# Mictronics/multi-sdr-gps-sim

Measured on AMD Instinct MI355X. Metric: IQ Msamples/s @16ch int8, higher is better.
Workload: dtype u64

## Files before the change

### multi-sdr-gps-sim_amd/csrc/gpsiq_chain_kernels.hip

```cpp
#include <hip/hip_runtime.h>

#include "gpsiq_internal.h"
#include "gpsiq_lane.h"

namespace gpsiq {

using lane::Prep;
using lane::Rec;
using lane::Stretch;
using lane::Walker;
using lane::u128;

constexpr int kPrepThreads = 1024;
constexpr int kLaneThreads = 256;
constexpr int kTabMinSeg = 16;

struct ScanR { u128 v; int flag; };
struct ScanD { double v; int flag; };
__device__ inline ScanR scan_join(const ScanR &p, ScanR a) { if (!a.flag) { a.v = p.v + a.v; a.flag = p.flag; } return a; }
__device__ inline ScanD scan_join(const ScanD &p, ScanD a) { if (!a.flag) { a.v = p.v + a.v; a.flag = p.flag; } return a; }
__device__ inline ScanR scan_up(const ScanR &x, int off)
{
    ScanR o;
    const uint64_t hi = __shfl_up((uint64_t) (x.v >> 64), off, 64), lo = __shfl_up((uint64_t) x.v, off, 64);
    o.v = ((u128) hi << 64) | lo; o.flag = __shfl_up(x.flag, off, 64);
    return o;
}
__device__ inline ScanD scan_up(const ScanD &x, int off) { ScanD o; o.v = __shfl_up(x.v, off, 64); o.flag = __shfl_up(x.flag, off, 64); return o; }
template <class S>
__device__ inline void block_scan(S mine, S *s_wave, S *before, S *total)
{
    const int lane = threadIdx.x & 63, wave = threadIdx.x >> 6, nwaves = (int) (blockDim.x >> 6);
    S inc = mine;
    for (int off = 1; off < 64; off <<= 1) {
        const S o = scan_up(inc, off);
        if (lane >= off) inc = scan_join(o, inc);
    }
    S exc = scan_up(inc, 1);
    if (lane == 0) { exc.v = 0; exc.flag = 0; }
    if (lane == 63) s_wave[wave] = inc;
    __syncthreads();
    S acc; acc.v = 0; acc.flag = 0;
    S mine_before = acc;
    for (int w = 0; w < nwaves; ++w) {
        if (w == wave) mine_before = acc;
        acc = scan_join(acc, s_wave[w]);
    }
    *before = scan_join(mine_before, exc);
    *total = acc;
    __syncthreads();
}

__global__ __launch_bounds__(kPrepThreads) void chain_prepare(const char *__restrict__ in_rows, int stride, int nblocks, int nchan, double delt, int nsamp,
                                                              const gpsiq_chain_est_t *__restrict__ start, Prep *__restrict__ prep,
                                                              double *__restrict__ c_before, gpsiq_chain_est_t *__restrict__ end)
{
    auto in_at = [&](size_t k) -> gpsiq_chain_in_t { return *reinterpret_cast<const gpsiq_chain_in_t *>(in_rows + k * (size_t) stride); };
    __shared__ ScanR s_wr[kPrepThreads / 64];
    __shared__ ScanD s_wd[kPrepThreads / 64];
    __shared__ int s_any_seed;
    const int i = blockIdx.x, tid = threadIdx.x;
    u128 Rc = 0;
    double Dc = 0.0, carr0 = 0.0, f_prev0 = 0.0;
    int prn0 = 0;
    bool exact0 = false;
    if (start) {
        const gpsiq_chain_est_t e = start[i];
        Rc = ((u128) e.r_hi << 64) | e.r_lo; Dc = e.drift; carr0 = e.carr; f_prev0 = e.f_carr; prn0 = e.prn; exact0 = (e.flags & GPSIQ_CHAIN_EXACT) != 0;
    }
    if (tid == 0) { c_before[i] = prn0 > 0 ? f_prev0 * delt : 0.0; s_any_seed = 0; }
    int last_prn = prn0;
    double last_f = f_prev0;
    __syncthreads();
    for (int base = 0; base < nblocks; base += kPrepThreads) {
        const int b = base + tid;
        const bool live = b < nblocks;
        gpsiq_chain_in_t d = {0.0, 0.0, 0, 0};
        int prev_prn = 0;
        if (live) {
            d = in_at((size_t) b * nchan + i);
            prev_prn = b > 0 ? in_at((size_t) (b - 1) * nchan + i).prn : prn0;
            if (prev_prn < 0) prev_prn = 0;
        }
        const bool active = live && d.prn > 0;
        const bool cont = active && b == 0 && exact0 && prev_prn == d.prn;
        const bool seed = active && (prev_prn != d.prn || cont);
        const double c = active ? d.f_carr * delt : 0.0;
        const double x_seed = cont ? carr0 : d.carr_phase;
        const u128 adv = active ? lane::advance_units(c, nsamp) : (u128) 0;
        ScanR mine;
        mine.flag = seed ? 1 : 0;
        mine.v = seed ? lane::phase_units(x_seed) + adv : adv;
        ScanR pr, er;
        block_scan(mine, s_wr, &pr, &er);
        const u128 R0 = seed ? lane::phase_units(x_seed) : pr.flag ? pr.v : Rc + pr.v;
        const double r0 = lane::units_to_double(R0);
        double core = 0.0;
        if (active && __builtin_fabs(c) < 0.5) core = lane::drift_core(c, seed ? (x_seed < 1.0 ? x_seed : 0.0) : r0, nsamp);
        ScanD md;
        md.flag = seed ? 1 : 0;
        md.v = core;
        ScanD pd, ed;
        block_scan(md, s_wd, &pd, &ed);
        const double D0 = seed ? 0.0 : pd.flag ? pd.v : Dc + pd.v;
        if (live) {
            Prep p = {0.0, 0.0, 0.0, lane::kSkip, 0};
            if (active) {
                p.c = c;
                p.est = seed ? x_seed : lane::wrap01(r0 + D0);
                p.core = core;
                p.flags = seed ? lane::kSeed : 0;
            }
            prep[(size_t) b * nchan + i] = p;
        }
        if (seed) atomicOr(&s_any_seed, 1);
        const int n_here = nblocks - base < kPrepThreads ? nblocks - base : kPrepThreads;
        __syncthreads();
        Rc = er.flag ? er.v : Rc + er.v;
        Dc = ed.flag ? ed.v : Dc + ed.v;
        {
            const gpsiq_chain_in_t l = in_at((size_t) (base + n_here - 1) * nchan + i);
            last_prn = l.prn > 0 ? l.prn : 0;
            last_f = l.f_carr;
        }
        __syncthreads();
    }
    if (end && tid == 0) {
        gpsiq_chain_est_t e;
        e.r_hi = (uint64_t) (Rc >> 64); e.r_lo = (uint64_t) Rc; e.drift = Dc; e.carr = 0.0; e.f_carr = last_f; e.prn = last_prn;
        e.flags = s_any_seed ? GPSIQ_CHAIN_RESEEDED : 0; e.first_prn = 0; e.reserved = 0;
        end[i] = e;
    }
}

template <int kSeg>
__global__ __launch_bounds__(kLaneThreads) void chain_lanes(const Prep *__restrict__ prep, const double *__restrict__ c_before,
                                                            int nblocks, int nchan, int nsamp, int max_seg, Rec *__restrict__ rec)
{
    constexpr int kBlocks = kLaneThreads / kSeg;
    __shared__ __attribute__((aligned(16))) unsigned char walker_raw[sizeof(Walker) * (kBlocks + 1)];
    Walker *walker = reinterpret_cast<Walker *>(walker_raw);
    constexpr int kEnt = kSeg >= kTabMinSeg ? lane::kEntriesHost : 0;
    __shared__ lane::Cycle cycles[kEnt ? kBlocks * kEnt : 1];
    __shared__ int usable[kBlocks + 1];
    const int groups = (nblocks + kBlocks - 1) / kBlocks;
    const int i = blockIdx.x / groups, b0 = (blockIdx.x % groups) * kBlocks;
    const int tid = threadIdx.x;
    if (tid <= kBlocks) {
        const int b = b0 - 1 + tid;
        double c = 0.0;
        if (b < 0) c = c_before[i];
        else if (b < nblocks) { const Prep p = prep[(size_t) b * nchan + i]; c = (p.flags & lane::kSkip) ? 0.0 : p.c; }
        const bool ok = c != 0.0 && __builtin_fabs(c) < 0.5;
        walker[tid].setup_head(ok ? c : 0.25);
        usable[tid] = ok && !walker[tid].general;
    }
    __syncthreads();
    for (int q = tid; q < (kBlocks + 1) * lane::kTab; q += kLaneThreads) {
        const int w = q / lane::kTab, s = q % lane::kTab;
        if (usable[w] && s > Walker::kLow && s <= (int) (1022 - walker[w].ec)) walker[w].setup_piece(s);
    }
    __syncthreads();
    const int blk = tid / kSeg, t = tid % kSeg, b = b0 + blk;
    const bool live = b < nblocks && usable[blk + 1];
    Prep p = {0.0, 0.0, 0.0, lane::kSkip, 0};
    if (live) p = prep[(size_t) b * nchan + i];
    const bool use_tab = live && kEnt > 0 && __builtin_fabs(p.c) * (double) nsamp > 2.0 * kEnt;
    if (use_tab) {
        for (int k = t; k < kEnt; k += kSeg) {
            lane::Cycle e;
            lane::build_cycle(walker[blk + 1], k, kEnt, &e);
            cycles[kEnt ? blk * kEnt + k : 0] = e;
        }
    }
    __syncthreads();
    int nseg = 0;
    Stretch st;
    st.r_in = 0.0; st.x_out = 0.0; st.x_end = 0.0; st.lo = 0; st.hi = 0; st.n_in = -1; st.n_out = -1; st.ok = 0; st.why = lane::kWhyAddend; st.sigma = 0; st.pad = 0;
    if (live) {
        nseg = lane::stretches(p.c, nsamp, max_seg < kSeg ? max_seg : kSeg);
        if (t < nseg) {
            const Walker *prev = (!(p.flags & lane::kSeed) && usable[blk]) ? &walker[blk] : nullptr;
            lane::walk_stretch(walker[blk + 1], prev, p, nsamp, t, nseg, use_tab ? &cycles[kEnt ? blk * kEnt : 0] : nullptr, kEnt, &st);
        }
    }
    const bool mine = live && t < nseg;
    const bool neg = walker[blk + 1].neg;
    const int64_t grid = neg ? 1 : 2;
    lane::JoinLane jl;
    jl.el = lane::join_identity(); jl.D = 0; jl.fail = 0; jl.pad = 0;
    Stretch before = st;
    before.x_out = __shfl_up(st.x_out, 1, kSeg); before.n_out = __shfl_up(st.n_out, 1, kSeg);
    if (mine) jl = lane::join_lane(before, st, t, grid);
    lane::JoinMap inc = jl.el;
    for (int off = 1; off < kSeg; off <<= 1) {
        lane::JoinMap o;
        o.t0 = __shfl_up(inc.t0, off, kSeg); o.t1 = __shfl_up(inc.t1, off, kSeg);
        if (t >= off) inc = lane::join_compose(o, inc);
    }
// ... 53 lines not shown
```

### multi-sdr-gps-sim_amd/csrc/gpsiq_eval.h

```cpp
#ifndef GPSIQ_EVAL_H
#define GPSIQ_EVAL_H

#include "../../include/gpsiq.h"
#include "gpsiq_lane.h"

namespace gpsiq {
namespace ev {

typedef unsigned __int128 u128;
typedef __int128 i128;

struct DChan {
    double   f_carr;
    double   carr_phase;
    int32_t  prn;
    uint32_t pos;
    double   f_code;
    double   code_phase;
    double   gain;
    uint64_t nav;
    double   start;
};
static_assert(sizeof(DChan) == 64, "DChan is one cache line");
constexpr uint32_t kBadPos = UINT32_C(1) << 31;
// ... 240 lines not shown
        if (c0 != c1) return false;
        if (c0 > (i128) INT64_MAX / 2 || c0 < -((i128) INT64_MAX / 2)) return false;
        *cell = (int64_t) c0;
        return true;
    }
};

enum { kEvalOk = 0, kEvalHost = 1 };
constexpr int kCandCap = 256;

GPSIQ_HD inline int eval_quantize(const DChan &d, double phase, double delt, int nsamp, gpsiq_qchan_t *q)
{
    if (d.prn > 0 && !(phase >= 0.0 && phase <= 1.0)) { gpsiq_qchan_t z; z.carr_phase = 0; z.carr_step = 0; z.code_frac = 0; z.code_step = 0; z.gain = 0.0; z.nav_bits = 0; z.chip0 = 0; z.icode = 0; z.prn = 0; *q = z; return kQStart; }
    const uint64_t seeded = phase_to_fixed(phase == 1.0 ? 0.0 : phase);
    return quantize_dchan(d, delt, nsamp, &seeded, q);
}

template <class Chips, class Emit>
GPSIQ_HD inline int eval_candidates(const DChan &d, const gpsiq_qchan_t &qq, double start, double delt, int nsamp, const Chips &chips, Emit &emit)
{
    const long ns = nsamp;
    if (ns <= 0 || d.prn <= 0) return kEvalOk;
    if (!(start >= 0.0 && start <= 1.0)) return -kQStart;
    const double carr_inc = d.f_carr * delt, code_inc = d.f_code * delt;
    uint64_t seed_off = (phase_to_fixed(start == 1.0 ? 0.0 : start) - qq.carr_phase) & kEvCarrMask;
    if (seed_off > (UINT64_C(1) << (GPSIQ_CARR_FRAC_BITS - 1))) seed_off = (UINT64_C(1) << GPSIQ_CARR_FRAC_BITS) - seed_off;
    const uint64_t w_carr = ((uint64_t) ns << (GPSIQ_CARR_FRAC_BITS - 54)) + (uint64_t) ns / 2 + 4 + seed_off;
    const uint64_t w_code = ((uint64_t) ns << (GPSIQ_CODE_FRAC_BITS - 44)) + (uint64_t) ns / 2 + 4;
    const bool want_c = carr_inc != 0.0 || seed_off != 0;
    if ((want_c && 2 * w_carr + 1 >= (UINT64_C(1) << (GPSIQ_CARR_FRAC_BITS - 9))) || 2 * w_code + 1 >= (UINT64_C(1) << GPSIQ_CODE_FRAC_BITS)) return kEvalHost;
    uint64_t nc = want_c ? next_candidate(qq.carr_phase, (uint64_t) qq.carr_step, GPSIQ_CARR_FRAC_BITS - 9, w_carr, ns, 0) : kNoHit;
    uint64_t nk = next_candidate(qq.code_frac, qq.code_step, GPSIQ_CODE_FRAC_BITS, w_code, ns, 0);
    if (nc == kNoHit && nk == kNoHit) return kEvalOk;
    DriftLite dc, dk;
    bool have_c = false, have_k = false;
    int count_c = 0, count_k = 0;
    const int icode = dchan_icode(d);
    while (nc != kNoHit || nk != kNoHit) {
        const uint64_t n = nc < nk ? nc : nk;
        const bool in_c = nc == n, in_k = nk == n;
        const uint64_t P = (qq.carr_phase + (uint64_t) qq.carr_step * n) & kEvCarrMask;
        const unsigned idx_f = (unsigned) (P >> (GPSIQ_CARR_FRAC_BITS - 9));
        const u128 T = (u128) qq.code_frac + (u128) qq.code_step * n;
        const uint64_t A = (uint64_t) qq.chip0 + (uint64_t) (T >> GPSIQ_CODE_FRAC_BITS);
        const unsigned chip_f = (unsigned) (A % GPSIQ_CA_SEQ_LEN);
        const long per_f = (long) (A / GPSIQ_CA_SEQ_LEN);
        const unsigned neg_f = chips(d.prn, chip_f) ^ dchan_nav_bit(d, ((long) icode + per_f) / 20);
        unsigned idx = idx_f, neg_d = neg_f;
        int64_t cell;
        if (in_c) {
            if (++count_c > kCandCap) return kEvalHost;
            if (!have_c) { dc.setup(carr_inc, 1, start); have_c = true; }
            if (!dc.cell_at((long) n, &cell)) return kEvalHost;
            idx = (unsigned) (cell & 511);
            nc = next_candidate(qq.carr_phase, (uint64_t) qq.carr_step, GPSIQ_CARR_FRAC_BITS - 9, w_carr, ns, (long) n + 1);
        }
        if (in_k) {
            if (++count_k > kCandCap) return kEvalHost;
            if (!have_k) { dk.setup(code_inc, 0, d.code_phase); have_k = true; }
            if (!dk.cell_at((long) n, &cell) || cell < 0) return kEvalHost;
            const unsigned chip_d = (unsigned) (cell % GPSIQ_CA_SEQ_LEN);
            const long per_d = (long) (cell / GPSIQ_CA_SEQ_LEN);
            neg_d = chips(d.prn, chip_d) ^ dchan_nav_bit(d, ((long) icode + per_d) / 20);
            nk = next_candidate(qq.code_frac, qq.code_step, GPSIQ_CODE_FRAC_BITS, w_code, ns, (long) n + 1);
        }
        if (idx != idx_f || neg_d != neg_f) emit((uint32_t) n, (uint16_t) idx, (uint8_t) neg_d);
    }
    return kEvalOk;
}

template <class Chips, class Emit>
GPSIQ_HD inline int eval_chan(const DChan &d, double start, double est, double delt, int nsamp, const Chips &chips, Emit &emit, gpsiq_qchan_t *q)
{
    const int qs = eval_quantize(d, est, delt, nsamp, q);
    if (qs != kQOk) return -qs;
    return eval_candidates(d, *q, start, delt, nsamp, chips, emit);
}

struct Link {
    int64_t t[4];
    int32_t abs;
    int32_t pad;
};
GPSIQ_HD inline Link link_identity() { Link l; l.t[0] = l.t[1] = l.t[2] = l.t[3] = 0; l.abs = 0; l.pad = 0; return l; }
GPSIQ_HD inline Link link_compose(const Link &a, const Link &b)
{
    if (b.abs) return b;
    Link o;
    o.abs = a.abs; o.pad = 0;
    for (int r = 0; r < 4; ++r) {
        const int64_t v = a.t[r];
        const int64_t at = a.abs ? v : (int64_t) r + v;
        o.t[r] = v + b.t[at & 3];
    }
    return o;
}
GPSIQ_HD inline int64_t link_apply(const Link &a, int64_t d) { return a.abs ? a.t[0] : d + a.t[d & 3]; }

GPSIQ_HD inline Link link_element(bool seed_or_unused, int64_t d0, const lane::Rec &prev, double xs, bool *ok)
{
    Link l = link_identity();
    *ok = true;
    if (seed_or_unused) { l.abs = 1; l.t[0] = l.t[1] = l.t[2] = l.t[3] = d0; return l; }
    int64_t J;
    const int64_t grid = prev.info & 0xff;
    if (!prev.ok || grid < 1 || grid > 2 || !lane::exact_units(prev.e, xs, &J)) { *ok = false; l.abs = 1; return l; }
    for (int r = 0; r < 4; ++r) l.t[r] = prev.cum[(r >> (grid - 1)) & 1] + J;
    return l;
}
GPSIQ_HD inline bool link_check(const lane::Rec &r, int64_t d, double *next)
{
    if (!r.ok) return false;
    const int64_t grid = r.info & 0xff;
    if (d < r.lo || d > r.hi || grid < 1 || grid > 2 || (d & (grid - 1))) return false;
    const int p = (int) ((d >> (grid - 1)) & 1);
    if (!(r.ok & (1 << p))) return false;
    double y;
    if (!lane::exact_shift(r.e, d + r.cum[p], &y) || !(y >= 0.0 && y < 1.0)) return false;
    *next = y;
    return true;
}

}
}
#endif
```

### multi-sdr-gps-sim_amd/csrc/gpsiq_eval_kernels.hip

```cpp
#include <hip/hip_runtime.h>

#include <cstdio>
#include <cstdlib>

#include "gpsiq_internal.h"
#include "gpsiq_eval.h"
#include "gpsiq_evalctl.h"

namespace gpsiq {

using ev::DChan;
using ev::Link;
using lane::Rec;

constexpr int kPackThreads = 128;
constexpr int kLinkThreads = 256;
constexpr int kEvalThreads = 128;

__device__ inline long long sum16(long long v)
{
    for (int off = 8; off >= 1; off >>= 1) v += __shfl_xor(v, off, 16);
    return v;
}
__device__ inline unsigned long long wave_max_u64(unsigned long long v)
{
    for (int off = 32; off >= 1; off >>= 1) { const unsigned long long o = __shfl_xor(v, off, 64); v = o > v ? o : v; }
    return v;
}
__device__ inline long long wave_max_i64(long long v)
{
    for (int off = 32; off >= 1; off >>= 1) { const long long o = __shfl_xor(v, off, 64); v = o > v ? o : v; }
    return v;
}

__device__ inline void reduce_params(bool counts, unsigned long long code_step, long long amp, EvalCtrl *ctrl)
{
    const long long blk_amp = sum16(counts ? amp : 0);
    const long long blk_active = sum16(counts ? 1 : 0);
    const unsigned long long ms = wave_max_u64(counts ? code_step : 0);
    const long long ma = wave_max_i64(blk_amp), mc = wave_max_i64(blk_active);
    if ((threadIdx.x & 63) == 0) {
        if (ms > __hip_atomic_load(&ctrl->max_code_step, __ATOMIC_RELAXED, __HIP_MEMORY_SCOPE_AGENT)) atomicMax(&ctrl->max_code_step, ms);
        if (ma > __hip_atomic_load(&ctrl->max_amp, __ATOMIC_RELAXED, __HIP_MEMORY_SCOPE_AGENT)) atomicMax(&ctrl->max_amp, ma);
        if ((int) mc > __hip_atomic_load(&ctrl->max_active, __ATOMIC_RELAXED, __HIP_MEMORY_SCOPE_AGENT)) atomicMax(&ctrl->max_active, (int) mc);
    }
}

constexpr int kPackRows = kPackThreads;
constexpr int kRowWords = (int) (sizeof(gpsiq_chan_t) / 8);
static_assert(sizeof(gpsiq_chan_t) % 8 == 0, "rows are streamed as 8-byte words");
__global__ __launch_bounds__(kPackThreads) void pack_raw(const gpsiq_chan_t *__restrict__ ch, int nblocks, int nchan, double delt,
                                                         DChan *__restrict__ out, EvalCtrl *__restrict__ ctrl)
{
    __shared__ __attribute__((aligned(16))) uint64_t rows[kPackRows * kRowWords];
    constexpr int kBlocksPerWg = kPackThreads / 16;
    const int blk0 = (int) blockIdx.x * kBlocksPerWg;
    const int nblk = nblocks - blk0 < kBlocksPerWg ? nblocks - blk0 : kBlocksPerWg;
    const size_t first = (size_t) blk0 * nchan;
    const int words = nblk > 0 ? nblk * nchan * kRowWords : 0;
    const uint64_t *src = reinterpret_cast<const uint64_t *>(ch + first);
    constexpr int kInFlight = 16;
    for (int w0 = threadIdx.x; w0 < words; w0 += kPackThreads * kInFlight) {
        uint64_t t[kInFlight];
#pragma unroll
        for (int j = 0; j < kInFlight; ++j) { const int w = w0 + j * kPackThreads; t[j] = w < words ? src[w] : 0; }
#pragma unroll
        for (int j = 0; j < kInFlight; ++j) { const int w = w0 + j * kPackThreads; if (w < words) rows[w] = t[j]; }
    }
    __syncthreads();
    const int lb = (int) (threadIdx.x >> 4), i = (int) (threadIdx.x & 15);
    const int b = blk0 + lb;
    const bool live = lb < nblk && i < nchan;
    DChan d;
    d.f_carr = 0.0; d.carr_phase = 0.0; d.prn = 0; d.pos = 0; d.f_code = 0.0; d.code_phase = 0.0; d.gain = 0.0; d.nav = 0; d.start = 0.0;
    if (live) {
        ev::pack_chan(*reinterpret_cast<const gpsiq_chan_t *>(&rows[(size_t) (lb * nchan + i) * kRowWords]), &d);
        out[(size_t) b * nchan + i] = d;
    }
    const double code_inc = d.f_code * delt;
    const bool counts = live && d.prn > 0 && d.prn <= 32 && code_inc > 0.0 && code_inc < 2.0 && d.gain > -ev::kEvMaxGain && d.gain < ev::kEvMaxGain;
    reduce_params(counts, counts ? (unsigned long long) (long long) __builtin_rint(code_inc * 0x1p56) : 0ull,
                  counts ? (long long) (250.0 * __builtin_fabs(d.gain)) : 0ll, ctrl);
}

__global__ __launch_bounds__(kLinkThreads) void chain_link_scan(DChan *__restrict__ chan, const Rec *__restrict__ rec, int b0, int nb, int nchan,
                                                                double delt, LinkCarry *__restrict__ carry, EvalCtrl *__restrict__ ctrl, int piece)
{
    __shared__ Link sl[kLinkThreads];
    __shared__ int s_seed[kLinkThreads], s_fail[kLinkThreads];
    __shared__ double s_next[kLinkThreads];
    __shared__ LinkCarry s_carry;
    __shared__ unsigned s_unknown, s_linked;
    const int i = blockIdx.x, tid = threadIdx.x;
    if (tid == 0) {
        LinkCarry c;
        c.d = 0; c.y = 0.0; c.prn = 0; c.known = 0;
        if (b0 > 0) c = carry[i];
        s_carry = c;
        s_unknown = 0; s_linked = 0;
    }
    __syncthreads();
    for (int base = 0; base < nb; base += kLinkThreads) {
        const int b = b0 + base + tid;
        const bool live = base + tid < nb;
        const LinkCarry cy = s_carry;
        const size_t at = (size_t) b * nchan + i;
        double carr_phase = 0.0, f_carr = 0.0;
        int prn = 0, prev_prn = 0;
        Rec r;
        r.xs = 0.0; r.e = 0.0; r.cum[0] = 0; r.cum[1] = 0; r.lo = 0; r.hi = 0; r.ok = 0; r.info = 0;
        if (live) {
            const DChan d = chan[at];
            carr_phase = d.carr_phase; f_carr = d.f_carr; prn = d.prn > 0 ? d.prn : 0;
            r = rec[at];
            if (b > 0) { const int p = chan[at - nchan].prn; prev_prn = p > 0 ? p : 0; }
        }
        const bool active = live && prn > 0;
        const bool seed = active && (b == 0 || prev_prn != prn);
        bool el_ok = true;
        Link el = ev::link_identity();
        if (live) {
            if (!active) el = ev::link_element(true, 0, r, 0.0, &el_ok);
            else if (seed) {
                int64_t d0 = 0;
                const bool ex = lane::exact_units(carr_phase, r.xs, &d0);
                el = ev::link_element(true, ex ? d0 : 0, r, 0.0, &el_ok);
                el_ok = ex;
            } else el = ev::link_element(false, 0, rec[at - nchan], r.xs, &el_ok);
        }
        sl[tid] = el;
        __syncthreads();
        for (int off = 1; off < kLinkThreads; off <<= 1) {
            Link a = sl[tid], p;
            const bool has = tid >= off;
            if (has) p = sl[tid - off];
            __syncthreads();
            if (has) sl[tid] = ev::link_compose(p, a);
            __syncthreads();
        }
        const int64_t dd = ev::link_apply(sl[tid], cy.d);
        double next = 0.0;
        const bool linked = active && el_ok && __builtin_fabs(f_carr * delt) < 0.5 && ev::link_check(r, dd, &next);
        s_seed[tid] = (live && (seed || !active)) ? tid : -1;
        s_fail[tid] = (active && !linked) ? tid : -1;
        s_next[tid] = next;
        __syncthreads();
        for (int off = 1; off < kLinkThreads; off <<= 1) {
            int a = s_seed[tid], f = s_fail[tid], pa = -1, pf = -1;
            const bool has = tid >= off;
            if (has) { pa = s_seed[tid - off]; pf = s_fail[tid - off]; }
            __syncthreads();
            if (has) { s_seed[tid] = pa > a ? pa : a; s_fail[tid] = pf > f ? pf : f; }
            __syncthreads();
        }
        int last_seed = s_seed[tid], last_fail = tid > 0 ? s_fail[tid - 1] : -2;
        if (last_seed < 0) last_seed = -1;
        if (last_fail < 0) last_fail = cy.known ? -2 : -1;
        const bool known = last_fail < last_seed;
        if (live) {
            double x = 0.0;
            if (active) x = seed ? carr_phase : (tid > 0 ? s_next[tid - 1] : cy.y);
            if (!active || known) chan[at].start = x;
            if (active && !(known && linked)) atomicAdd(&s_unknown, 1u);
            if (active && known && linked) atomicAdd(&s_linked, 1u);
        }
        const int n_here = nb - base < kLinkThreads ? nb - base : kLinkThreads;
        __syncthreads();
        if (tid == n_here - 1) {
            LinkCarry c;
            c.d = dd; c.y = next; c.prn = prn; c.known = (active && known && linked) ? 1 : 0;
            s_carry = c;
        }
        __syncthreads();
    }
    if (tid == 0) {
        carry[i] = s_carry;
        ctrl->unknown[piece][i] = (int) s_unknown;
        atomicAdd(&ctrl->linked, s_linked);
    }
}

__global__ __launch_bounds__(256) void gather_slot(const DChan *__restrict__ chan, const Rec *__restrict__ rec, int b0, int nb, int nchan, int slot,
                                                   EvalSlotRow *__restrict__ out)
{
    const int k = (int) (blockIdx.x * 256u + threadIdx.x);
    if (k >= nb) return;
    const size_t at = (size_t) (b0 + k) * nchan + slot;
    const DChan d = chan[at];
    EvalSlotRow r;
    r.f_carr = d.f_carr; r.carr_phase = d.carr_phase; r.start = d.start; r.prn = d.prn; r.pad = 0;
    const Rec m = rec[at];
    r.map.xs = m.xs; r.map.e = m.e; r.map.cum[0] = m.cum[0]; r.map.cum[1] = m.cum[1]; r.map.lo = m.lo; r.map.hi = m.hi; r.map.ok = m.ok; r.map.info = m.info;
    out[k] = r;
}
__global__ __launch_bounds__(256) void scatter_starts(DChan *__restrict__ chan, int b0, int nb, int nchan, int slot, const double *__restrict__ starts)
{
    const int k = (int) (blockIdx.x * 256u + threadIdx.x);
    if (k < nb) chan[(size_t) (b0 + k) * nchan + slot].start = starts[k];
}

struct DevChips {
    const DeviceTables *tab;
    __device__ unsigned operator()(int prn, unsigned chip) const { return (tab->prn_ext[prn - 1][chip >> 5] >> (chip & 31)) & 1u; }
};
struct DevEmit {
    gpsiq_patch_t *patches; unsigned cap; EvalCtrl *ctrl; uint32_t block; uint8_t slot;
    __device__ void operator()(uint32_t sample, uint16_t lut, uint8_t neg)
    {
        const unsigned k = atomicAdd(&ctrl->npatch, 1u);
        if (k < cap) { gpsiq_patch_t p; p.block = block; p.sample = sample; p.slot = slot; p.neg = neg; p.lut = lut; patches[k] = p; }
    }
};

__device__ inline void report_error(EvalCtrl *ctrl, size_t flat, int status)
{
    atomicMin(&ctrl->err_key, ((unsigned long long) flat << 8) | (unsigned long long) (status & 0xff));
}

__device__ inline int store_compacted(gpsiq_qchan_t *__restrict__ qout, size_t row, int i, int nchan, bool active, const gpsiq_qchan_t &q)
{
    const unsigned long long m = __ballot(active);
    const unsigned bits = (unsigned) (m >> (threadIdx.x & 48)) & 0xffffu;
    const int slot = __popc(bits & ((1u << i) - 1u)), na = __popc(bits);
    if (active) qout[row + slot] = q;
    if (i >= na && i < nchan) {
        gpsiq_qchan_t z;
        z.carr_phase = 0; z.carr_step = 0; z.code_frac = 0; z.code_step = 0; z.gain = 0.0; z.nav_bits = 0; z.chip0 = 0; z.icode = 0; z.prn = 0;
        qout[row + i] = z;
    }
// ... 242 lines not shown
```

### multi-sdr-gps-sim_amd/csrc/gpsiq_tile_body.inc

```
    constexpr int kLutEntries = BOTH ? 1024 : 512;
    constexpr int LFMT = LEVEL ? GPSIQ_SC16 : FMT;
    static_assert(!LEVEL || (NOISE && !BOTH), "the level stage follows the noise in the noise kernels");
    constexpr int kThreads = WAVES * 64;
    __shared__ uint32_t lut[NCH][kLutEntries];
    __shared__ uint32_t ext[NCH][kPrnExtWords];
    __shared__ uint32_t win[WAVES][ROWS * H][NCH];
    __shared__ gpsiq_qchan_t qs[NCH];
    static_assert(H == 1 || H == 2, "one window per row or per half row");
    static_assert(!BOTH || FAST, "the both-polarity table is a form of the plain-add core");
    static_assert(kLutEntries % kThreads == 0 || kThreads % kLutEntries == 0, "LUT build: whole passes");
    constexpr int kSpan = 64 / H;

    const int tid = threadIdx.x;
    int blk, tile;
    if ((int) blockIdx.x < big_wgs) {
        blk = blockIdx.x / tiles_per_block; tile = blockIdx.x % tiles_per_block;
    } else {
        const int r = (int) blockIdx.x - big_wgs;
        blk = big_blocks + r / tiles_small; tile = r % tiles_small;
        wave_rows = ROWS;
    }
    const gpsiq_qchan_t *q_blk = desc + (size_t) (block0 + blk) * nchan;
    const int nq = nchan < NCH ? nchan : NCH;
    for (int i = tid; i < NCH * 12; i += kThreads)
// ... 8 lines not shown
            const double g = qs[c].gain;
            const int ts = (int) (sk * g), tc = (int) (ck * g);
            constexpr int kPre = LFMT == GPSIQ_SC08 ? 4 : 0;
            if (FAST && LFMT == GPSIQ_SC08)
                lut[c][e] = (((uint32_t) tc & 0xfffu) << 4) | ((uint32_t) ts << 20);
            else if (FAST)
                lut[c][e] = (uint32_t) (tc + ts * 65536) + (c == 0 ? 0x8000u : 0u);
            else      lut[c][e] = (((uint32_t) tc << kPre) & 0xffffu) | ((uint32_t) ts << (16 + kPre));
        }
    }
    for (int e = tid; e < NCH * kPrnExtWords; e += kThreads) {
        const int c = e / kPrnExtWords, w = e % kPrnExtWords;
        ext[c][w] = qs[c].prn ? tab->prn_ext[qs[c].prn - 1][w] : 0u;
    }
    [[maybe_unused]] const noise::Entry *nz = nullptr;
    if constexpr (NOISE) {
        __shared__ noise::Entry nz_s[noise::kTabEntries];
        for (int e = tid; e < noise::kTabEntries; e += kThreads) nz_s[e] = ntab[e];
        nz = nz_s;
    }
    __syncthreads();
    uint8_t *blk_dst = dst + (size_t) blk * block_stride;

    const int wave = tid >> 6, lane = tid & 63;
    const uint32_t wave_samples = (uint32_t) wave_rows * 64u;
    const uint32_t n_wave = ((uint32_t) tile * WAVES + (uint32_t) wave) * wave_samples;
    if (n_wave >= (uint32_t) nsamp) return;
    [[maybe_unused]] uint64_t nx = 0;
    if constexpr (NOISE) {
        uint64_t A, C;
        noise::jump((uint32_t) __builtin_amdgcn_readfirstlane((int) (n_wave >> 6)), noise::kMul, noise::kInc, &A, &C);
        nx = A * noise::lane_start(nseed, nblock0 + (uint64_t) (block0 + blk), (uint32_t) lane) + C;
    }

    constexpr int kPad = NCH <= 4 ? 4 : NCH <= 8 ? 8 : 16;
    constexpr int kGroups = 64 / kPad;
    constexpr int kRun = ROWS * H / kGroups;
    static_assert((ROWS * H) % kGroups == 0, "windows per chunk must split over the lane groups");
    const int c_raw = lane % kPad, wg = lane / kPad;
    const int wc = c_raw < NCH ? c_raw : 0;
    const bool w_store = c_raw < NCH;
    uint32_t w_k, w_nrev, w_nrot, w_dint;
    int32_t w_e1;
    uint64_t w_fr, w_dfr;
    {
        const gpsiq_qchan_t &q = qs[wc];
        const uint32_t n_row = n_wave + (uint32_t) wg * (uint32_t) kSpan;
        const unsigned __int128 T = (unsigned __int128) q.code_frac +
                                    (unsigned __int128) q.code_step * (unsigned __int128) n_row;
        const uint32_t A = (uint32_t) q.chip0 + (uint32_t) (uint64_t) (T >> GPSIQ_CODE_FRAC_BITS);
        w_fr = (uint64_t) T & kCodeFracMask;
        w_k = A % GPSIQ_CA_SEQ_LEN;
        const uint32_t ic = q.icode + A / GPSIQ_CA_SEQ_LEN;
        w_e1 = (int32_t) ((20u - ic % 20u) * GPSIQ_CA_SEQ_LEN - w_k) - 1;
        w_nrev = __builtin_bitreverse32(q.nav_bits >> ((ic / 20u) & 31u));
        w_nrot = 0u - A;
        const unsigned __int128 step = (unsigned __int128) q.code_step * (unsigned) (kSpan * kGroups);
        w_dint = (uint32_t) (uint64_t) (step >> GPSIQ_CODE_FRAC_BITS);
        w_dfr = (uint64_t) step & kCodeFracMask;
    }

    const uint32_t n0 = n_wave + (uint32_t) lane;
    uint64_t P[NCH], Q[NCH], dP[NCH], dQ[NCH];
#pragma unroll
    for (int c = 0; c < NCH; ++c) {
        const bool have = c < nchan;
        const uint64_t p0 = have ? q_blk[c].carr_phase : 0u, ps = have ? (uint64_t) q_blk[c].carr_step : 0u;
        const uint64_t f0 = have ? q_blk[c].code_frac : 0u, cs = have ? q_blk[c].code_step : 0u;
        const uint64_t c0 = have ? (uint64_t) q_blk[c].chip0 : 0u;
        constexpr int kAlign = BOTH ? 64 - GPSIQ_CARR_FRAC_BITS : 0;
        P[c] = (p0 + ps * (uint64_t) n0) << kAlign;
        Q[c] = (c0 << GPSIQ_CODE_FRAC_BITS) + f0 + cs * (uint64_t) n0;
        dP[c] = (ps * 64u) << kAlign;
        dQ[c] = cs * 64u;
    }

    const unsigned char *lut_b = reinterpret_cast<const unsigned char *>(&lut[0][0]);
    const uint32_t *w_row = &win[wave][H == 2 ? lane >> 5 : 0][0];
    uint32_t *w_dst = &win[wave][wg][wc];

    [[maybe_unused]] int32_t l_neg = 0;
    if constexpr (LEVEL && FAST) asm("v_mov_b32 %0, %1" : "=v"(l_neg) : "s"(-(int32_t) lqmax));

    auto row_body = [&](int r, uint32_t n_chunk, bool check) {
        uint32_t iq;
        [[maybe_unused]] uint32_t zi = 0, zq = 0;
        if constexpr (NOISE) {
            const uint32_t w = noise::xsh_rr(nx);
            nx = nx * noise::kMul + noise::kInc;
            zi = (uint32_t) noise::z(nz, w & 0xffffu);
            zq = (uint32_t) noise::z(nz, w >> 16);
        }
        if (FAST) {
            uint32_t sum = 0u;
#pragma unroll
            for (int c = 0; c < NCH; ++c) {
                const uint32_t w = w_row[r * (H * NCH) + c];
                const uint32_t t = w >> ((uint32_t) (Q[c] >> 56) & 31u);
                if (BOTH) {
                    const uint32_t x = __builtin_amdgcn_alignbit(t, (uint32_t) (P[c] >> 32), 21u);
                    sum += *reinterpret_cast<const uint32_t *>(lut_b + c * 4096 + (x & 0xffcu));
                } else {
                    const uint32_t x = (t << 26) + (uint32_t) (P[c] >> 32);
                    const uint32_t a = (x >> 16) & 0x7fcu;
                    sum += *reinterpret_cast<const uint32_t *>(lut_b + c * 2048 + a);
                }
                P[c] += dP[c];
                Q[c] += dQ[c];
            }
            if constexpr (NOISE && !LEVEL) {
                if (FMT == GPSIQ_SC08)
                    sum = (sum & ~0xf0000u) + ((zi & 0xfffu) << 4) + (zq << 20);
                else
                    sum += zi + (zq << 16);
            }
            iq = LFMT == GPSIQ_SC16 ? sum ^ 0x8000u : sum;
        } else {
            s16x2 acc0 = (s16x2) (0), acc1 = (s16x2) (0);
#pragma unroll
            for (int c = 0; c < NCH; ++c) {
                const uint32_t w = w_row[r * (H * NCH) + c];
                const uint32_t b = (uint32_t) (Q[c] >> 56);
                const uint32_t m = (uint32_t) __builtin_amdgcn_sbfe((int) w, b, 1u);
                const uint32_t sgn = m | 0x00010001u;
                const uint32_t a = (uint32_t) (P[c] >> 48) & 0x7fcu;
                const uint32_t v = *reinterpret_cast<const uint32_t *>(lut_b + c * 2048 + a);
                if (c & 1) acc1 = __builtin_bit_cast(s16x2, v) * __builtin_bit_cast(s16x2, sgn) + acc1;
                else       acc0 = __builtin_bit_cast(s16x2, v) * __builtin_bit_cast(s16x2, sgn) + acc0;
                P[c] += dP[c];
                Q[c] += dQ[c];
            }
            if constexpr (NOISE && !LEVEL) {
                constexpr int kPre = FMT == GPSIQ_SC08 ? 4 : 0;
                acc0 = __builtin_bit_cast(s16x2, ((zi << kPre) & 0xffffu) | (zq << (16 + kPre))) + acc0;
            }
            iq = __builtin_bit_cast(uint32_t, acc0 + acc1);
        }
        if constexpr (LEVEL) {
            const int32_t ai = (int32_t) (int16_t) iq + (int32_t) zi, aq = ((int32_t) iq >> 16) + (int32_t) zq;
            const int32_t yi = (int32_t) (((int64_t) ai * (int64_t) (int32_t) lmult + 32768) >> 16);
            const int32_t yq = (int32_t) (((int64_t) aq * (int64_t) (int32_t) lmult + 32768) >> 16);
            uint32_t oi, oq;
            if constexpr (!FAST) l_neg = -(int32_t) lqmax;
            asm("v_med3_i32 %0, %1, %2, %3" : "=v"(oi) : "v"(yi), "v"(l_neg), "s"((int32_t) lqmax));
            asm("v_med3_i32 %0, %1, %2, %3" : "=v"(oq) : "v"(yq), "v"(l_neg), "s"((int32_t) lqmax));
            const uint32_t n = n_chunk + (uint32_t) lane + (uint32_t) r * 64u;
            if (!check || n < (uint32_t) nsamp) {
                if (FMT == GPSIQ_SC16) *reinterpret_cast<uint32_t *>(blk_dst + n * 4u) = (oi & 0xffffu) | (oq << 16);
                else *reinterpret_cast<uint16_t *>(blk_dst + n * 2u) = (uint16_t) ((oi & 0xffu) | (oq << 8));
            }
            return;
        }
        const uint32_t n = n_chunk + (uint32_t) lane + (uint32_t) r * 64u;
        if (!check || n < (uint32_t) nsamp) {
            if (FMT == GPSIQ_SC16)
                *reinterpret_cast<uint32_t *>(blk_dst + n * 4u) = iq;
            else
                *reinterpret_cast<uint16_t *>(blk_dst + n * 2u) = (uint16_t) __builtin_amdgcn_perm(iq, iq, 0x0c0c0301u);
        }
    };

    for (int row0 = 0; row0 < wave_rows; row0 += ROWS) {
        const uint32_t n_chunk = n_wave + (uint32_t) row0 * 64u;
        constexpr int kGrp = 4;
        static_assert(kRun % kGrp == 0, "window groups");
        const uint32_t reach = (uint32_t) kGrp * (w_dint + 1u) + 32u;
#pragma unroll 1
        for (int i0 = 0; i0 < kRun; i0 += kGrp) {
            if (__builtin_amdgcn_ballot_w64((uint32_t) w_e1 <= reach) == 0) {
                const uint32_t nrot0 = w_nrot;
                const uint32_t d0 = (uint32_t) ((int32_t) w_nrev >> 31);
#pragma unroll
                for (int i = i0; i < i0 + kGrp; ++i) {
                    const uint32_t lo = ext[wc][w_k >> 5], hi = ext[wc][(w_k >> 5) + 1];
                    const uint32_t S = __builtin_amdgcn_alignbit(hi, lo, w_k) ^ d0;
                    if (w_store) w_dst[i * (kGroups * NCH)] = __builtin_amdgcn_alignbit(S, S, w_nrot);
                    w_fr += w_dfr;
                    const uint32_t adv = w_dint + (uint32_t) (w_fr >> GPSIQ_CODE_FRAC_BITS);
                    w_fr &= kCodeFracMask;
                    w_nrot -= adv;
                    const uint32_t k2 = w_k + adv;
                    w_k = k2 - GPSIQ_CA_SEQ_LEN < k2 ? k2 - GPSIQ_CA_SEQ_LEN : k2;
                }
                w_e1 -= (int32_t) (nrot0 - w_nrot);
            } else {
#pragma unroll
                for (int i = i0; i < i0 + kGrp; ++i) {
                    const uint32_t lo = ext[wc][w_k >> 5], hi = ext[wc][(w_k >> 5) + 1];
                    uint32_t S = __builtin_amdgcn_alignbit(hi, lo, w_k);
                    S ^= (uint32_t) ((int32_t) w_nrev >> 31);
                    const bool edge = (uint32_t) w_e1 < 31u;
                    if (__builtin_expect(__builtin_amdgcn_ballot_w64(edge) != 0, 0)) {
                        if (edge && ((w_nrev ^ (w_nrev << 1)) >> 31)) S ^= 0xfffffffeu << w_e1;
                    }
                    if (w_store) w_dst[i * (kGroups * NCH)] = __builtin_amdgcn_alignbit(S, S, w_nrot);
                    w_fr += w_dfr;
                    const uint32_t adv = w_dint + (uint32_t) (w_fr >> GPSIQ_CODE_FRAC_BITS);
                    w_fr &= kCodeFracMask;
                    w_nrot -= adv;
                    const uint32_t k2 = w_k + adv;
                    w_k = k2 - GPSIQ_CA_SEQ_LEN < k2 ? k2 - GPSIQ_CA_SEQ_LEN : k2;
                    const int32_t e = w_e1 - (int32_t) adv;
                    const int32_t m = e >> 31;
                    w_e1 = e + (m & (int32_t) (20 * GPSIQ_CA_SEQ_LEN));
                    w_nrev <<= (uint32_t) m & 1u;
                }
            }
        }
        __builtin_amdgcn_fence(__ATOMIC_RELEASE, "workgroup");
        __builtin_amdgcn_wave_barrier();
        __builtin_amdgcn_fence(__ATOMIC_ACQUIRE, "workgroup");

        int rows = wave_rows - row0;
        rows = rows < ROWS ? rows : ROWS;
        if (n_chunk + (uint32_t) rows * 64u <= (uint32_t) nsamp) {
            const int rows_s = __builtin_amdgcn_readfirstlane(rows);
#pragma clang loop unroll(disable) vectorize(disable) interleave(disable)
            for (int r = 0; r < rows_s; ++r) row_body(r, n_chunk, false);
        } else {
            const int in_block = (int) (((uint32_t) nsamp - n_chunk + 63u) >> 6);
            rows = rows < in_block ? rows : in_block;
#pragma clang loop unroll(disable) vectorize(disable) interleave(disable)
            for (int r = 0; r < rows; ++r) row_body(r, n_chunk, true);
        }
        __builtin_amdgcn_fence(__ATOMIC_RELEASE, "workgroup");
        __builtin_amdgcn_wave_barrier();
        __builtin_amdgcn_fence(__ATOMIC_ACQUIRE, "workgroup");
    }
```

Before: 376,500.

## Process four blocks per thread in chain_prepare and cap register use in link scan

chain_prepare now runs 256 threads per block, each handling four consecutive blocks. The phase scan is reduced per thread first, and the drift scan becomes a custom 16-lane group scan over four elements per thread, which cuts block_scan width and barrier cost. Both chain_prepare and chain_link_scan get amdgpu_waves_per_eu hints. Indexed Link table lookups are replaced with select-based pick4/pick2 so the arrays stay in registers instead of scratch, and the scan loops are kept rolled to limit register pressure. This adds serial work per thread and reduces parallelism per block.

```diff
diff --git a/multi-sdr-gps-sim_amd/csrc/gpsiq_chain_kernels.hip b/multi-sdr-gps-sim_amd/csrc/gpsiq_chain_kernels.hip
--- a/multi-sdr-gps-sim_amd/csrc/gpsiq_chain_kernels.hip
+++ b/multi-sdr-gps-sim_amd/csrc/gpsiq_chain_kernels.hip
@@ -11,7 +11,10 @@
 using lane::Walker;
 using lane::u128;
 
-constexpr int kPrepThreads = 1024;
+constexpr int kPrepRound = 1024;
+constexpr int kPrepPer = 4;
+constexpr int kPrepThreads = kPrepRound / kPrepPer;
+constexpr int kPrepWavesPerEu = 5;
 constexpr int kLaneThreads = 256;
 constexpr int kTabMinSeg = 16;
 
@@ -51,13 +54,51 @@
     __syncthreads();
 }
 
-__global__ __launch_bounds__(kPrepThreads) void chain_prepare(const char *__restrict__ in_rows, int stride, int nblocks, int nchan, double delt, int nsamp,
-                                                              const gpsiq_chain_est_t *__restrict__ start, Prep *__restrict__ prep,
-                                                              double *__restrict__ c_before, gpsiq_chain_est_t *__restrict__ end)
+constexpr int kPrepGroup = 64 / kPrepPer;
+static_assert(kPrepPer == 4 && kPrepGroup == 16, "drift_scan spells the steps of 1 and 2 lanes out for four blocks per thread");
+__device__ inline ScanD scan_up_group(const ScanD &x, int off) { ScanD o; o.v = __shfl_up(x.v, off, kPrepGroup); o.flag = __shfl_up(x.flag, off, kPrepGroup); return o; }
+__device__ inline void drift_scan(const ScanD (&mine)[kPrepPer], ScanD *s_wave, ScanD (&before)[kPrepPer], ScanD *total)
+{
+    const int u = threadIdx.x % kPrepGroup, row = threadIdx.x / kPrepGroup;
+    ScanD x0 = mine[0], x1 = mine[1], x2 = mine[2], x3 = mine[3];
+    {
+        const ScanD o = scan_up_group(x3, 1);
+        const ScanD n0 = u >= 1 ? scan_join(o, x0) : x0, n1 = scan_join(x0, x1), n2 = scan_join(x1, x2), n3 = scan_join(x2, x3);
+        x0 = n0; x1 = n1; x2 = n2; x3 = n3;
+    }
+    {
+        const ScanD o2 = scan_up_group(x2, 1), o3 = scan_up_group(x3, 1);
+        const ScanD n0 = u >= 1 ? scan_join(o2, x0) : x0, n1 = u >= 1 ? scan_join(o3, x1) : x1, n2 = scan_join(x0, x2), n3 = scan_join(x1, x3);
+        x0 = n0; x1 = n1; x2 = n2; x3 = n3;
+    }
+    for (int m = 1; m < kPrepGroup; m <<= 1) {
+        const ScanD o0 = scan_up_group(x0, m), o1 = scan_up_group(x1, m), o2 = scan_up_group(x2, m), o3 = scan_up_group(x3, m);
+        if (u >= m) { x0 = scan_join(o0, x0); x1 = scan_join(o1, x1); x2 = scan_join(o2, x2); x3 = scan_join(o3, x3); }
+    }
+    ScanD e0 = scan_up_group(x3, 1);
+    if (u == 0) { e0.v = 0; e0.flag = 0; }
+    if (u == kPrepGroup - 1) s_wave[row] = x3;
+    __syncthreads();
+    ScanD acc; acc.v = 0; acc.flag = 0;
+    ScanD mine_before = acc;
+    for (int w = 0; w < kPrepRound / 64; ++w) {
+        if (w == row) mine_before = acc;
+        acc = scan_join(acc, s_wave[w]);
+    }
+    before[0] = scan_join(mine_before, e0); before[1] = scan_join(mine_before, x0);
+    before[2] = scan_join(mine_before, x1); before[3] = scan_join(mine_before, x2);
+    *total = acc;
+    __syncthreads();
+}
+
+__global__ __launch_bounds__(kPrepThreads) __attribute__((amdgpu_waves_per_eu(kPrepWavesPerEu)))
+void chain_prepare(const char *__restrict__ in_rows, int stride, int nblocks, int nchan, double delt, int nsamp,
+                   const gpsiq_chain_est_t *__restrict__ start, Prep *__restrict__ prep,
+                   double *__restrict__ c_before, gpsiq_chain_est_t *__restrict__ end)
 {
     auto in_at = [&](size_t k) -> gpsiq_chain_in_t { return *reinterpret_cast<const gpsiq_chain_in_t *>(in_rows + k * (size_t) stride); };
     __shared__ ScanR s_wr[kPrepThreads / 64];
-    __shared__ ScanD s_wd[kPrepThreads / 64];
+    __shared__ ScanD s_wd[kPrepRound / 64];
     __shared__ int s_any_seed;
     const int i = blockIdx.x, tid = threadIdx.x;
     u128 Rc = 0;
@@ -72,49 +113,72 @@
     int last_prn = prn0;
     double last_f = f_prev0;
     __syncthreads();
-    for (int base = 0; base < nblocks; base += kPrepThreads) {
-        const int b = base + tid;
-        const bool live = b < nblocks;
-        gpsiq_chain_in_t d = {0.0, 0.0, 0, 0};
+    for (int base = 0; base < nblocks; base += kPrepRound) {
+        const int b0 = base + tid * kPrepPer;
+        double c[kPrepPer], xs[kPrepPer];
+        bool active[kPrepPer], seed[kPrepPer];
         int prev_prn = 0;
-        if (live) {
-            d = in_at((size_t) b * nchan + i);
-            prev_prn = b > 0 ? in_at((size_t) (b - 1) * nchan + i).prn : prn0;
+        if (b0 < nblocks) {
+            prev_prn = b0 > 0 ? in_at((size_t) (b0 - 1) * nchan + i).prn : prn0;
             if (prev_prn < 0) prev_prn = 0;
         }
-        const bool active = live && d.prn > 0;
-        const bool cont = active && b == 0 && exact0 && prev_prn == d.prn;
-        const bool seed = active && (prev_prn != d.prn || cont);
-        const double c = active ? d.f_carr * delt : 0.0;
-        const double x_seed = cont ? carr0 : d.carr_phase;
-        const u128 adv = active ? lane::advance_units(c, nsamp) : (u128) 0;
-        ScanR mine;
-        mine.flag = seed ? 1 : 0;
-        mine.v = seed ? lane::phase_units(x_seed) + adv : adv;
+        auto phase_element = [&](int k) -> ScanR {
+            ScanR m;
+            m.flag = seed[k] ? 1 : 0;
+            m.v = active[k] ? lane::advance_units(c[k], nsamp) : (u128) 0;
+            if (seed[k]) m.v += lane::phase_units(xs[k]);
+            return m;
+        };
+        bool any_seed = false;
+        ScanR all; all.v = 0; all.flag = 0;
+#pragma unroll
+        for (int k = 0; k < kPrepPer; ++k) {
+            const int b = b0 + k;
+            gpsiq_chain_in_t d = {0.0, 0.0, 0, 0};
+            if (b < nblocks) d = in_at((size_t) b * nchan + i);
+            active[k] = b < nblocks && d.prn > 0;
+            const bool cont = active[k] && b == 0 && exact0 && prev_prn == d.prn;
+            seed[k] = active[k] && (prev_prn != d.prn || cont);
+            c[k] = active[k] ? d.f_carr * delt : 0.0;
+            xs[k] = cont ? carr0 : d.carr_phase;
+            all = scan_join(all, phase_element(k));
+            any_seed |= seed[k];
+            prev_prn = d.prn < 0 ? 0 : d.prn;
+        }
         ScanR pr, er;
-        block_scan(mine, s_wr, &pr, &er);
-        const u128 R0 = seed ? lane::phase_units(x_seed) : pr.flag ? pr.v : Rc + pr.v;
-        const double r0 = lane::units_to_double(R0);
-        double core = 0.0;
-        if (active && __builtin_fabs(c) < 0.5) core = lane::drift_core(c, seed ? (x_seed < 1.0 ? x_seed : 0.0) : r0, nsamp);
-        ScanD md;
-        md.flag = seed ? 1 : 0;
-        md.v = core;
-        ScanD pd, ed;
-        block_scan(md, s_wd, &pd, &ed);
-        const double D0 = seed ? 0.0 : pd.flag ? pd.v : Dc + pd.v;
-        if (live) {
-            Prep p = {0.0, 0.0, 0.0, lane::kSkip, 0};
-            if (active) {
-                p.c = c;
-                p.est = seed ? x_seed : lane::wrap01(r0 + D0);
-                p.core = core;
-                p.flags = seed ? lane::kSeed : 0;
+        block_scan(all, s_wr, &pr, &er);
+#pragma unroll
+        for (int k = 0; k < kPrepPer; ++k) {
+            const ScanR m = phase_element(k);
+            if (!seed[k]) xs[k] = lane::units_to_double(pr.flag ? pr.v : Rc + pr.v);
+            pr = scan_join(pr, m);
+        }
+        ScanD md[kPrepPer], pd[kPrepPer], ed;
+#pragma unroll
+        for (int k = 0; k < kPrepPer; ++k) {
+            double core = 0.0;
+            if (active[k] && __builtin_fabs(c[k]) < 0.5) core = lane::drift_core(c[k], seed[k] && !(xs[k] < 1.0) ? 0.0 : xs[k], nsamp);
+            md[k].flag = seed[k] ? 1 : 0;
+            md[k].v = core;
+        }
+        drift_scan(md, s_wd, pd, &ed);
+#pragma unroll
+        for (int k = 0; k < kPrepPer; ++k) {
+            const int b = b0 + k;
+            const double D0 = seed[k] ? 0.0 : pd[k].flag ? pd[k].v : Dc + pd[k].v;
+            if (b < nblocks) {
+                Prep p = {0.0, 0.0, 0.0, lane::kSkip, 0};
+                if (active[k]) {
+                    p.c = c[k];
+                    p.est = seed[k] ? xs[k] : lane::wrap01(xs[k] + D0);
+                    p.core = md[k].v;
+                    p.flags = seed[k] ? lane::kSeed : 0;
+                }
+                prep[(size_t) b * nchan + i] = p;
             }
-            prep[(size_t) b * nchan + i] = p;
-        }
-        if (seed) atomicOr(&s_any_seed, 1);
-        const int n_here = nblocks - base < kPrepThreads ? nblocks - base : kPrepThreads;
+        }
+        if (any_seed) atomicOr(&s_any_seed, 1);
+        const int n_here = nblocks - base < kPrepRound ? nblocks - base : kPrepRound;
         __syncthreads();
         Rc = er.flag ? er.v : Rc + er.v;
         Dc = ed.flag ? ed.v : Dc + ed.v;
diff --git a/multi-sdr-gps-sim_amd/csrc/gpsiq_eval.h b/multi-sdr-gps-sim_amd/csrc/gpsiq_eval.h
--- a/multi-sdr-gps-sim_amd/csrc/gpsiq_eval.h
+++ b/multi-sdr-gps-sim_amd/csrc/gpsiq_eval.h
@@ -346,6 +346,13 @@
     int32_t abs;
     int32_t pad;
 };
+GPSIQ_HD inline int64_t pick4(const int64_t (&t)[4], int64_t k)
+{
+    const int64_t t0 = t[0], t1 = t[1], t2 = t[2], t3 = t[3];
+    const int64_t lo = (k & 1) ? t1 : t0, hi = (k & 1) ? t3 : t2;
+    return (k & 2) ? hi : lo;
+}
+GPSIQ_HD inline int64_t pick2(const int64_t (&t)[2], int64_t k) { const int64_t t0 = t[0], t1 = t[1]; return (k & 1) ? t1 : t0; }
 GPSIQ_HD inline Link link_identity() { Link l; l.t[0] = l.t[1] = l.t[2] = l.t[3] = 0; l.abs = 0; l.pad = 0; return l; }
 GPSIQ_HD inline Link link_compose(const Link &a, const Link &b)
 {
@@ -355,11 +362,11 @@
     for (int r = 0; r < 4; ++r) {
         const int64_t v = a.t[r];
         const int64_t at = a.abs ? v : (int64_t) r + v;
-        o.t[r] = v + b.t[at & 3];
+        o.t[r] = v + pick4(b.t, at);
     }
     return o;
 }
-GPSIQ_HD inline int64_t link_apply(const Link &a, int64_t d) { return a.abs ? a.t[0] : d + a.t[d & 3]; }
+GPSIQ_HD inline int64_t link_apply(const Link &a, int64_t d) { return a.abs ? a.t[0] : d + pick4(a.t, d); }
 
 GPSIQ_HD inline Link link_element(bool seed_or_unused, int64_t d0, const lane::Rec &prev, double xs, bool *ok)
 {
@@ -369,7 +376,7 @@
     int64_t J;
     const int64_t grid = prev.info & 0xff;
     if (!prev.ok || grid < 1 || grid > 2 || !lane::exact_units(prev.e, xs, &J)) { *ok = false; l.abs = 1; return l; }
-    for (int r = 0; r < 4; ++r) l.t[r] = prev.cum[(r >> (grid - 1)) & 1] + J;
+    for (int r = 0; r < 4; ++r) l.t[r] = pick2(prev.cum, r >> (grid - 1)) + J;
     return l;
 }
 GPSIQ_HD inline bool link_check(const lane::Rec &r, int64_t d, double *next)
@@ -380,7 +387,7 @@
     const int p = (int) ((d >> (grid - 1)) & 1);
     if (!(r.ok & (1 << p))) return false;
     double y;
-    if (!lane::exact_shift(r.e, d + r.cum[p], &y) || !(y >= 0.0 && y < 1.0)) return false;
+    if (!lane::exact_shift(r.e, d + pick2(r.cum, p), &y) || !(y >= 0.0 && y < 1.0)) return false;
     *next = y;
     return true;
 }
diff --git a/multi-sdr-gps-sim_amd/csrc/gpsiq_eval_kernels.hip b/multi-sdr-gps-sim_amd/csrc/gpsiq_eval_kernels.hip
--- a/multi-sdr-gps-sim_amd/csrc/gpsiq_eval_kernels.hip
+++ b/multi-sdr-gps-sim_amd/csrc/gpsiq_eval_kernels.hip
@@ -15,6 +15,7 @@
 
 constexpr int kPackThreads = 128;
 constexpr int kLinkThreads = 256;
+constexpr int kLinkWavesPerEu = 5;
 constexpr int kEvalThreads = 128;
 
 __device__ inline long long sum16(long long v)
@@ -83,8 +84,9 @@
                   counts ? (long long) (250.0 * __builtin_fabs(d.gain)) : 0ll, ctrl);
 }
 
-__global__ __launch_bounds__(kLinkThreads) void chain_link_scan(DChan *__restrict__ chan, const Rec *__restrict__ rec, int b0, int nb, int nchan,
-                                                                double delt, LinkCarry *__restrict__ carry, EvalCtrl *__restrict__ ctrl, int piece)
+__global__ __launch_bounds__(kLinkThreads) __attribute__((amdgpu_waves_per_eu(kLinkWavesPerEu)))
+void chain_link_scan(DChan *__restrict__ chan, const Rec *__restrict__ rec, int b0, int nb, int nchan,
+                     double delt, LinkCarry *__restrict__ carry, EvalCtrl *__restrict__ ctrl, int piece)
 {
     __shared__ Link sl[kLinkThreads];
     __shared__ int s_seed[kLinkThreads], s_fail[kLinkThreads];
@@ -130,6 +132,7 @@
         }
         sl[tid] = el;
         __syncthreads();
+#pragma unroll 1
         for (int off = 1; off < kLinkThreads; off <<= 1) {
             Link a = sl[tid], p;
             const bool has = tid >= off;
@@ -145,6 +148,7 @@
         s_fail[tid] = (active && !linked) ? tid : -1;
         s_next[tid] = next;
         __syncthreads();
+#pragma unroll 1
         for (int off = 1; off < kLinkThreads; off <<= 1) {
             int a = s_seed[tid], f = s_fail[tid], pa = -1, pf = -1;
             const bool has = tid >= off;
```

Result: no change. 376,500, median of 2 (+0.0%).

## Software-pipeline fast row loop in four-row trips with vector window prefetch

Applied to the files above, without the earlier changes.

Adds a trip loop for the fast core that processes four rows per iteration. It reads the per-channel window words as 16-byte vectors and prefetches the next row's windows while the current row's LUT gathers are in flight, with sched_barriers separating the shift, gather and accumulate phases. Noise, formatting and store code is factored into shared lambdas so the old per-row path still handles leftover rows and tail chunks. The goal is to hide LDS latency and cut per-row loop overhead, at the cost of more registers (arrays t, g and wv of NCH entries), which may lower occupancy.

```diff
diff --git a/multi-sdr-gps-sim_amd/csrc/gpsiq_tile_body.inc b/multi-sdr-gps-sim_amd/csrc/gpsiq_tile_body.inc
--- a/multi-sdr-gps-sim_amd/csrc/gpsiq_tile_body.inc
+++ b/multi-sdr-gps-sim_amd/csrc/gpsiq_tile_body.inc
@@ -114,15 +114,100 @@
     [[maybe_unused]] int32_t l_neg = 0;
     if constexpr (LEVEL && FAST) asm("v_mov_b32 %0, %1" : "=v"(l_neg) : "s"(-(int32_t) lqmax));
 
+    constexpr uint32_t kElem = FMT == GPSIQ_SC16 ? 4u : 2u;
+
+    auto noise_row = [&](uint32_t &zi, uint32_t &zq) {
+        const uint32_t w = noise::xsh_rr(nx);
+        nx = nx * noise::kMul + noise::kInc;
+        zi = (uint32_t) noise::z(nz, w & 0xffffu);
+        zq = (uint32_t) noise::z(nz, w >> 16);
+    };
+    auto fast_word = [&](uint32_t sum, uint32_t zi, uint32_t zq) -> uint32_t {
+        if constexpr (NOISE && !LEVEL) {
+            if (FMT == GPSIQ_SC08)
+                sum = (sum & ~0xf0000u) + ((zi & 0xfffu) << 4) + (zq << 20);
+            else
+                sum += zi + (zq << 16);
+        }
+        return LFMT == GPSIQ_SC16 ? sum ^ 0x8000u : sum;
+    };
+    auto emit = [&](uint32_t iq, [[maybe_unused]] uint32_t zi, [[maybe_unused]] uint32_t zq, uint8_t *o, bool ok) {
+        if constexpr (LEVEL) {
+            const int32_t ai = (int32_t) (int16_t) iq + (int32_t) zi, aq = ((int32_t) iq >> 16) + (int32_t) zq;
+            const int32_t yi = (int32_t) (((int64_t) ai * (int64_t) (int32_t) lmult + 32768) >> 16);
+            const int32_t yq = (int32_t) (((int64_t) aq * (int64_t) (int32_t) lmult + 32768) >> 16);
+            uint32_t oi, oq;
+            if constexpr (!FAST) l_neg = -(int32_t) lqmax;
+            asm("v_med3_i32 %0, %1, %2, %3" : "=v"(oi) : "v"(yi), "v"(l_neg), "s"((int32_t) lqmax));
+            asm("v_med3_i32 %0, %1, %2, %3" : "=v"(oq) : "v"(yq), "v"(l_neg), "s"((int32_t) lqmax));
+            if (ok) {
+                if (FMT == GPSIQ_SC16) *reinterpret_cast<uint32_t *>(o) = (oi & 0xffffu) | (oq << 16);
+                else *reinterpret_cast<uint16_t *>(o) = (uint16_t) ((oi & 0xffu) | (oq << 8));
+            }
+        } else if (ok) {
+            if (FMT == GPSIQ_SC16)
+                *reinterpret_cast<uint32_t *>(o) = iq;
+            else
+                *reinterpret_cast<uint16_t *>(o) = (uint16_t) __builtin_amdgcn_perm(iq, iq, 0x0c0c0301u);
+        }
+    };
+
+    constexpr int kTrip = FAST && !(NOISE && NCH > 12) ? 4 : 1;
+    static_assert(ROWS % kTrip == 0, "whole trips in a full chunk");
+    static_assert(NCH % 4 == 0, "window words are read four at a time");
+    typedef uint32_t win4 __attribute__((ext_vector_type(4)));
+    auto read_windows = [&](const uint32_t *w, uint32_t (&wv)[NCH]) {
+        const win4 *w4 = reinterpret_cast<const win4 *>(__builtin_assume_aligned(w, 16));
+#pragma unroll
+        for (int c = 0; c < NCH; c += 4) {
+            const win4 v = w4[c / 4];
+            wv[c] = v.x; wv[c + 1] = v.y; wv[c + 2] = v.z; wv[c + 3] = v.w;
+        }
+    };
+    [[maybe_unused]] auto trip_body = [&](const uint32_t *&w_at, uint32_t (&wv)[NCH], uint8_t *o, int w_step) {
+#pragma unroll
+        for (int j = 0; j < kTrip; ++j) {
+            uint32_t t[NCH], g[NCH];
+            [[maybe_unused]] uint32_t zi = 0, zq = 0;
+#pragma unroll
+            for (int c = 0; c < NCH; ++c) t[c] = wv[c] >> ((uint32_t) (Q[c] >> 56) & 31u);
+            __builtin_amdgcn_sched_barrier(0);
+#pragma unroll
+            for (int c = 0; c < NCH; ++c) {
+                if (BOTH) {
+                    const uint32_t x = __builtin_amdgcn_alignbit(t[c], (uint32_t) (P[c] >> 32), 21u);
+                    g[c] = *reinterpret_cast<const uint32_t *>(lut_b + c * 4096 + (x & 0xffcu));
+                } else {
+                    const uint32_t x = (t[c] << 26) + (uint32_t) (P[c] >> 32);
+                    g[c] = *reinterpret_cast<const uint32_t *>(lut_b + c * 2048 + ((x >> 16) & 0x7fcu));
+                }
+            }
+            __builtin_amdgcn_sched_barrier(0);
+            if constexpr (NOISE) noise_row(zi, zq);
+#pragma unroll
+            for (int c = 0; c < NCH; ++c) {
+                if (c == NCH / 2) {
+                    __builtin_amdgcn_sched_barrier(0);
+                    if (j + 1 == kTrip) w_at += w_step;
+                    read_windows(j + 1 == kTrip ? w_at : w_at + (j + 1) * (H * NCH), wv);
+                    __builtin_amdgcn_sched_barrier(0);
+                }
+                P[c] += dP[c];
+                Q[c] += dQ[c];
+                asm("" : "+v"(P[c]), "+v"(Q[c]));
+            }
+            __builtin_amdgcn_sched_barrier(0);
+            uint32_t sum = 0u;
+#pragma unroll
+            for (int c = 0; c < NCH; ++c) sum += g[c];
+            emit(fast_word(sum, zi, zq), zi, zq, o + (uint32_t) j * (64u * kElem), true);
+        }
+    };
+
     auto row_body = [&](int r, uint32_t n_chunk, bool check) {
         uint32_t iq;
         [[maybe_unused]] uint32_t zi = 0, zq = 0;
-        if constexpr (NOISE) {
-            const uint32_t w = noise::xsh_rr(nx);
-            nx = nx * noise::kMul + noise::kInc;
-            zi = (uint32_t) noise::z(nz, w & 0xffffu);
-            zq = (uint32_t) noise::z(nz, w >> 16);
-        }
+        if constexpr (NOISE) noise_row(zi, zq);
         if (FAST) {
             uint32_t sum = 0u;
 #pragma unroll
@@ -140,13 +225,7 @@
                 P[c] += dP[c];
                 Q[c] += dQ[c];
             }
-            if constexpr (NOISE && !LEVEL) {
-                if (FMT == GPSIQ_SC08)
-                    sum = (sum & ~0xf0000u) + ((zi & 0xfffu) << 4) + (zq << 20);
-                else
-                    sum += zi + (zq << 16);
-            }
-            iq = LFMT == GPSIQ_SC16 ? sum ^ 0x8000u : sum;
+            iq = fast_word(sum, zi, zq);
         } else {
             s16x2 acc0 = (s16x2) (0), acc1 = (s16x2) (0);
 #pragma unroll
@@ -168,28 +247,8 @@
             }
             iq = __builtin_bit_cast(uint32_t, acc0 + acc1);
         }
-        if constexpr (LEVEL) {
-            const int32_t ai = (int32_t) (int16_t) iq + (int32_t) zi, aq = ((int32_t) iq >> 16) + (int32_t) zq;
-            const int32_t yi = (int32_t) (((int64_t) ai * (int64_t) (int32_t) lmult + 32768) >> 16);
-            const int32_t yq = (int32_t) (((int64_t) aq * (int64_t) (int32_t) lmult + 32768) >> 16);
-            uint32_t oi, oq;
-            if constexpr (!FAST) l_neg = -(int32_t) lqmax;
-            asm("v_med3_i32 %0, %1, %2, %3" : "=v"(oi) : "v"(yi), "v"(l_neg), "s"((int32_t) lqmax));
-            asm("v_med3_i32 %0, %1, %2, %3" : "=v"(oq) : "v"(yq), "v"(l_neg), "s"((int32_t) lqmax));
-            const uint32_t n = n_chunk + (uint32_t) lane + (uint32_t) r * 64u;
-            if (!check || n < (uint32_t) nsamp) {
-                if (FMT == GPSIQ_SC16) *reinterpret_cast<uint32_t *>(blk_dst + n * 4u) = (oi & 0xffffu) | (oq << 16);
-                else *reinterpret_cast<uint16_t *>(blk_dst + n * 2u) = (uint16_t) ((oi & 0xffu) | (oq << 8));
-            }
-            return;
-        }
         const uint32_t n = n_chunk + (uint32_t) lane + (uint32_t) r * 64u;
-        if (!check || n < (uint32_t) nsamp) {
-            if (FMT == GPSIQ_SC16)
-                *reinterpret_cast<uint32_t *>(blk_dst + n * 4u) = iq;
-            else
-                *reinterpret_cast<uint16_t *>(blk_dst + n * 2u) = (uint16_t) __builtin_amdgcn_perm(iq, iq, 0x0c0c0301u);
-        }
+        emit(iq, zi, zq, blk_dst + n * kElem, !check || n < (uint32_t) nsamp);
     };
 
     for (int row0 = 0; row0 < wave_rows; row0 += ROWS) {
@@ -247,8 +306,24 @@
         rows = rows < ROWS ? rows : ROWS;
         if (n_chunk + (uint32_t) rows * 64u <= (uint32_t) nsamp) {
             const int rows_s = __builtin_amdgcn_readfirstlane(rows);
+            int r = 0;
+            if constexpr (kTrip > 1) {
+                const int trips = rows_s / kTrip;
+                if (trips > 0) {
+                    const uint32_t *w_at = w_row;
+                    uint32_t wv[NCH];
+                    read_windows(w_at, wv);
+                    uint32_t o_off = (n_chunk + (uint32_t) lane) * kElem;
 #pragma clang loop unroll(disable) vectorize(disable) interleave(disable)
-            for (int r = 0; r < rows_s; ++r) row_body(r, n_chunk, false);
+                    for (int t = trips; t > 0; --t) {
+                        trip_body(w_at, wv, blk_dst + o_off, t > 1 ? kTrip * (H * NCH) : 0);
+                        o_off += (uint32_t) kTrip * 64u * kElem;
+                    }
+                    r = trips * kTrip;
+                }
+            }
+#pragma clang loop unroll(disable) vectorize(disable) interleave(disable)
+            for (; r < rows_s; ++r) row_body(r, n_chunk, false);
         } else {
             const int in_block = (int) (((uint32_t) nsamp - n_chunk + 63u) >> 6);
             rows = rows < in_block ? rows : in_block;
```

Result: faster. 380,600 before, 389,200 after, median of 6 (+2.2%).
